# halajun/diasss

Measured on AMD Instinct MI355X. Metric: sonar frames/sec end-to-end (extract+match+LM solve), higher is better.
Workload: dtype u8/int32 (extract, match) + f64 (geo gate, LM); 1 GPU; 200 synthetic 2000x1024 frames, dense all-pairs; frames=200, pings=2000, bins=1024, pairs=19900

## Files before the change

### diasss_amd/csrc/dsss_pg.hip

```cpp
#include "dsss_internal.h"
#include "dsss_lm.h"
#include <utility>
#include "dsss_pg_kernels.h"
#include <algorithm>
#include <numeric>
#include <random>
#include <cstdlib>
#include <chrono>
#include <thread>
#include <mutex>
#include <future>

namespace {

struct pg_dev {
    dsss_ctx* ctx = nullptr;
    int rc = DSSS_OK;
    static constexpr size_t CHUNK = (size_t)256 << 20;
    template <typename T> int alloc(dsss_ctx* c, T** p, size_t n) { void* q = nullptr; if (!rc) rc = grab(c, &q, std::max<size_t>(n, 1) * sizeof(T)); *p = (T*)q; return rc; }
    int grab(dsss_ctx* c, void** p, size_t n) {
        if (!ctx) { ctx = c; c->pg_chunk_cur = 0; c->pg_chunk_off = 0; }
        const size_t bytes = (n + 255) & ~(size_t)255;
        for (;;) {
            if (c->pg_chunk_cur < c->pg_chunks.size()) {
// ... 454 lines not shown
        dv.alloc(c, &d_L, nnzL * 36); dv.alloc(c, &d_ubin, (size_t)S.ubin_doubles);
        if (dv.alloc(c, &d_aval, (size_t)nval * 36 + comm_total)) return dv.rc;
        d_comm = d_aval + (size_t)nval * 36; d_avalif = d_comm; d_xif = d_comm + ncv * 36; d_commU = d_xif + nif * 6;
        if (A.local) ifslot.swap(A.ifslot_g);
        else { ifslot.assign(ns, -1); for (size_t q = 0; q < nif; ++q) ifslot[S.iface_seps[q]] = (int)q; }
        dv.later(&d_ifslot, ifslot); dv.later(&d_ifsep, A.local ? A.ifsep_g : S.iface_seps);
        dv.later(&d_binptr, S.binptr); dv.later(&d_bincols, S.bincols); dv.later(&d_binperm, S.bin_perm);
        dv.later(&d_dest, A.local ? A.dest_g : S.dest_bin);
        dv.later(&d_binroot_ptr, S.binroot_ptr); dv.later(&d_binroot_idx, S.binroot_idx); dv.later(&d_broot_b, S.broot_b); dv.later(&d_broot_uoff, S.broot_uoff);
        dv.later(&d_broot_of_col, S.broot_of_col);
        if (dv.flush(c, st)) return dv.rc;
        { const int nb_all = (int)S.binptr.size() - 1, sel_lo = A.local ? 0 : part_lo, sel_hi = A.local ? 1 : part_hi;
          bin_lo = 0; while (bin_lo < nb_all && S.bin_part[bin_lo] < sel_lo) ++bin_lo; bin_hi = bin_lo; while (bin_hi < nb_all && S.bin_part[bin_hi] < sel_hi) ++bin_hi; }
        nbins = bin_hi - bin_lo;
        return DSSS_OK;
    }
    void bottom_trial(double bins_flops) {
        hipMemsetAsync(d_L, 0, nnzL * 36 * sizeof(double), st);
        if (nparts > 1) hipMemsetAsync(d_comm, 0, comm_total * sizeof(double), st);
        hipLaunchKernelGGL(pg_scatter_base_kernel, dim3((unsigned)(((long long)ns * 78 + 255) / 256)), dim3(256), 0, st, ns, d_t2, d_perm, d_D1, d_g1, d_s2DL, d_s2DR, d_s2GL, d_s2GR, d_s2S, d_dest, d_L, d_aval, d_x,
                           d_ifslot, d_avalif, d_xif, kp0, kp1);
        if (ne > 0) hipLaunchKernelGGL(pg_scatter_lc_kernel, dim3((unsigned)(((long long)ne * 36 + 255) / 256)), dim3(256), 0, st, n, ne, ns, d_Ji, d_ew, d_dest, d_L, d_aval, d_avalif, d_eo, mp0, mp1, d_lc_link);
        if (nbins > 0) { dsss_scope s1(c, DSSS_K_PG_SUBTREE, bins_flops);
                         hipLaunchKernelGGL(pg_factor_subtree_kernel, dim3(nbins), dim3(256), 0, st, d_binperm + bin_lo, d_binptr, d_bincols, d_colptr, d_rlptr, d_rlcol, d_rlpos, d_mapptr, d_map, d_L, d_x, d_fail,
                                            d_binroot_ptr, d_binroot_idx, d_broot_b, d_broot_uoff, d_broot_of_col, d_anc_first, d_anc_rel, d_ubin, d_rdiag); }
    }
    int join_analysis() {
        sym_thread.join();
        if (S.ownership_violations) DSSS_FAIL(c, DSSS_E_STATE, "pose-graph analysis: %d separators with a higher-rank neighbour are not interface", S.ownership_violations);
        return DSSS_OK;
    }

    int upload_fronts() {
        if (!pre_bins) {
            if (const int rc = upload_lists()) return rc;
            if (const int rc = upload_bottom()) return rc;
        } else if (c->prof.on) c->prof.work[DSSS_K_PG_SUBTREE] += std::max(0.0, S.flops_factor - S.flops_fronts);
        if (sw.opt.verbose)
            fprintf(stderr, "[dsss pg] rank %d/%d parts %d (own %d..%d, poses %d..%d)  %s analysis of %d separators  poses %d  LC edges %d  separators %d "
                    "(interface %zu)  nnz(L) blocks %zu  bins %d (%d cols)  fronts %d (largest %d block rows, arena %.0f MB)  panels %d in %d levels  "
                    "all-reduce %.1f MB\n", rank, world, nparts, part_lo, part_hi, mp0, mp1, A.local ? "rank-local" : "replicated", S.ns, n, ne, ns,
                    S.iface_seps.size(), nnzL, (int)S.binptr.size() - 1, (int)S.bincols.size(), (int)S.f_c0.size(), S.max_front_n, S.front_doubles * 8e-6,
                    S.npanels, S.nlev, (S.comm_doubles + 36.0 * S.comm_vals.size() + 6.0 * S.iface_seps.size()) * 8e-6);
        const int nfr = (int)S.f_c0.size();
        f_if = A.local && !S.iface_seps.empty() ? nfr - 1 : -1;
        if_ld = f_if >= 0 ? (size_t)S.f_ld[f_if] : 0; if_count = if_ld * if_ld + if_ld;
        if (f_if >= 0 && (S.f_part[f_if] != -1 || S.f_off[f_if] + (long long)(if_ld * if_ld) != S.front_doubles))
// ... 478 lines not shown
```

### diasss_amd/csrc/dsss_pg_bins.hip

```cpp
#include "dsss_pg_kernels.h"
#include "dsss_pg_dev.h"
#pragma clang fp contract(fast)
__global__ __launch_bounds__(256) void pg_build_map_kernel(int nupd, const int* __restrict__ rlrow, const int* __restrict__ rlptr,
                                                           const int* __restrict__ rlcol, const int* __restrict__ rlpos,
                                                           const int* __restrict__ colptr, const int* __restrict__ rowidx,
                                                           const long long* __restrict__ mapptr, int* __restrict__ upd_map, const int* __restrict__ nupd_dev)
{
    const int e = blockIdx.x * 256 + threadIdx.x;
    if (e >= (nupd_dev ? *nupd_dev : nupd)) return;
    const int j = rlrow[e], k = rlcol[e];
    const int c0 = colptr[j], m = colptr[j + 1] - c0;
    int* mp = upd_map + mapptr[j] + (long long)(e - rlptr[j]) * m;
    int q = 0;
    for (int p = rlpos[e]; p < colptr[k + 1]; ++p) {
        const int i = rowidx[p];
        while (q < m && rowidx[c0 + q] < i) ++q;
        if (q < m && rowidx[c0 + q] == i) mp[q] = p;
    }
}

__global__ __launch_bounds__(256) void pg_rl_count_kernel(int ns, const int* __restrict__ colptr, const int* __restrict__ rowidx, const char* __restrict__ binned,
                                                          int* __restrict__ cnt)
{
    const int k = blockIdx.x * 256 + threadIdx.x;
// ... 99 lines not shown
#pragma unroll
            for (int c = 0; c < 6; ++c) a[u][c] = Lik[c];
        }
#pragma unroll
        for (int u = 0; u < 4; ++u) {
            if (pos[u] < 0) continue;
            const double* B = s_Ljk + (t + u) * 36;
#pragma unroll
            for (int s = 0; s < 6; ++s)
                acc[s] += a[u][0] * B[s * 6] + a[u][1] * B[s * 6 + 1] + a[u][2] * B[s * 6 + 2] + a[u][3] * B[s * 6 + 3] + a[u][4] * B[s * 6 + 4] + a[u][5] * B[s * 6 + 5];
        }
    }
    for (; t < tn; ++t) {
        const int pos = mp[(size_t)t * m];
        if (pos < 0) continue;
        const double* Lik = Lvals + (size_t)pos * 36 + r * 6;
        const double* B = s_Ljk + t * 36;
        const double a0 = Lik[0], a1 = Lik[1], a2 = Lik[2], a3 = Lik[3], a4 = Lik[4], a5 = Lik[5];
#pragma unroll
        for (int s = 0; s < 6; ++s)
            acc[s] += a0 * B[s * 6] + a1 * B[s * 6 + 1] + a2 * B[s * 6 + 2] + a3 * B[s * 6 + 3] + a4 * B[s * 6 + 4] + a5 * B[s * 6 + 5];
    }
}
__global__ __launch_bounds__(256) void pg_factor_subtree_kernel(const int* __restrict__ bin_perm, const int* __restrict__ binptr, const int* __restrict__ bincols,
                                                                const int* __restrict__ colptr, const int* __restrict__ rlptr,
                                                                const int* __restrict__ rlcol, const int* __restrict__ rlpos,
                                                                const long long* __restrict__ mapptr, const int* __restrict__ upd_map,
                                                                double* __restrict__ Lvals, double* __restrict__ x, int* __restrict__ fail,
                                                                const int* __restrict__ binroot_ptr, const int* __restrict__ binroot_idx,
                                                                const int* __restrict__ broot_b, const long long* __restrict__ broot_uoff,
                                                                const int* __restrict__ broot_of_col, const int* __restrict__ anc_first,
                                                                const int* __restrict__ anc_rel, double* __restrict__ ubin, double* __restrict__ rdiag)
{
    __shared__ double s_Ljk[PG_TCH * 36];
    __shared__ double s_yk[PG_TCH * 6];
    __shared__ double s_diag[36];
    __shared__ int s_arel[48];
    __shared__ double s_ri[6];
    __shared__ double s_y[6];
    __shared__ double s_xj[6];
    __shared__ int s_ok;
    const int bin = bin_perm[blockIdx.x];
    for (int q = binroot_ptr[bin]; q < binroot_ptr[bin + 1]; ++q) {
        const int ri = binroot_idx[q]; const long long b6 = 6LL * broot_b[ri]; double* U = ubin + broot_uoff[ri];
        for (long long e = threadIdx.x; e < b6 * b6 + b6; e += 256) U[e] = 0.0;
    }
    struct colinfo { int j, c0, m, t0, T, af, ri, b6; long long mapoff, uoff; };
// ... 105 lines not shown
            double* __restrict__ g = U + (size_t)b6 * b6;
            if ((int)threadIdx.x < ta) s_arel[threadIdx.x] = anc_rel[c0 + af + threadIdx.x];
            __syncthreads();
            if ((int)threadIdx.x < 6 * ta) {
                const int pa = threadIdx.x / 6, a = threadIdx.x - pa * 6;
                const double* La = s_Ljk + pa * 36 + a * 6;
                g[s_arel[pa] * 6 + a] -= La[0] * s_y[0] + La[1] * s_y[1] + La[2] * s_y[2] + La[3] * s_y[3] + La[4] * s_y[4] + La[5] * s_y[5];
            }
            const int npair = ta * (ta + 1) / 2;
            for (int e = threadIdx.x; e < 36 * npair; e += 256) {
                const int pr = e / 36, ab = e - 36 * pr;
                int pa = (int)((sqrtf(8.0f * (float)pr + 1.0f) - 1.0f) * 0.5f);
                while (pa * (pa + 1) / 2 > pr) --pa;
                while ((pa + 1) * (pa + 2) / 2 <= pr) ++pa;
                const int pb = pr - pa * (pa + 1) / 2, a = ab / 6, b = ab - 6 * a;
                const double* La = s_Ljk + pa * 36 + a * 6; const double* Lb = s_Ljk + pb * 36 + b * 6;
                U[(size_t)(s_arel[pa] * 6 + a) * b6 + s_arel[pb] * 6 + b] -= La[0] * Lb[0] + La[1] * Lb[1] + La[2] * Lb[2] + La[3] * Lb[3] + La[4] * Lb[4] + La[5] * Lb[5];
            }
        }
        __syncthreads();
        __threadfence_block();
    }
}
__global__ __launch_bounds__(64) void pg_bwd_subtree_kernel(const int* __restrict__ bin_perm, const int* __restrict__ binptr, const int* __restrict__ bincols,
                                                            const int* __restrict__ colptr, const int* __restrict__ rowidx,
                                                            const double* __restrict__ Lvals, double* __restrict__ x, const double* __restrict__ rdiag)
{
    const int lane = threadIdx.x;
    const int bin = bin_perm[blockIdx.x];
    const int ci_lo = binptr[bin];
    int jn = 0, cn0 = 0, cn1 = 0;
    double ldn[36], rin[6];
    auto ahead = [&](int ci2) {
        jn = bincols[ci2]; cn0 = colptr[jn]; cn1 = colptr[jn + 1];
        if (lane == 0) {
            const double* Ld = Lvals + (size_t)cn0 * 36;
#pragma unroll
            for (int a = 0; a < 36; ++a) ldn[a] = Ld[a];
#pragma unroll
            for (int a = 0; a < 6; ++a) rin[a] = rdiag[(size_t)jn * 6 + a];
        }
    };
    if (binptr[bin + 1] - 1 >= ci_lo) ahead(binptr[bin + 1] - 1);
    for (int ci = binptr[bin + 1] - 1; ci >= ci_lo; --ci) {
        const int j = jn, c0 = cn0, c1 = cn1;
        double ld[36], ri[6];
// ... 36 lines not shown
```

### diasss_amd/csrc/dsss_pg_kernels.h

```cpp
#pragma once
#include "dsss_internal.h"
#include "dsss_pose.h"
#include "dsss_pg_sym.h"

struct pg_weights { double prior[6], odo[6]; };

struct pg_pack { const double* U; const double* g; double* dst; int cld, cb; };
struct pg_front {
    long long off, roff;
    int ld, n6, s6, c0;
    int rowptr, pan0;
    int ch0, ch1, fa0, fa1;
};
struct pg_child { const double* U; const double* g; long long relptr; int cld, cb; };

#define PG_ASM_POSES 32
#define PG_NB4 24
#define PG_RSU_MAX_TILES 320
#define PG_RSU32_MAX_TILES 80
#define PG_BWD2_LD 97
#define PG_BWD2_SX 8192
#define PG_BWD_SPLIT 2048
#define PG_BWD_RC 512
#define RNG_PER_THREAD 16
// ... 16 lines not shown
__global__ void pg_flag_blocksum_kernel(const int* __restrict__ flags, long long n, int* __restrict__ bsum);
__global__ void pg_flag_scan_kernel(int* __restrict__ bsum, int nb, int* __restrict__ total);
__global__ void pg_flag_compact_kernel(const int* __restrict__ flags, const double* __restrict__ pairs, long long n, const int* __restrict__ bsum, long long need_pairs, double* __restrict__ normals);
__global__ void lc_edge_compact_kernel(const int* __restrict__ flags, const int* __restrict__ bsum, const unsigned long long* __restrict__ slot, int total, const int* __restrict__ kp7_off, const double* __restrict__ kp7,
                                       const dsss_lc* __restrict__ lcs, const int* __restrict__ act_s, const int* __restrict__ frame_off, int cap, dsss_lc_edge* __restrict__ edges, int2* __restrict__ ab);
__global__ void pg_gather_dr_kernel(const unsigned long long* __restrict__ fptr, const int* __restrict__ foff, double* __restrict__ out);
__global__ void pg_gather_pose_kernel(int n, const int* __restrict__ idx, const pose_t* __restrict__ X, pose_t* __restrict__ out);
__global__ void pg_sep_xy_kernel(int ns, const int* __restrict__ sep_pose, const double* __restrict__ dr6, double* __restrict__ xy);
__global__ void pg_init_kernel(int n, const double* __restrict__ dr6, const double* __restrict__ normals, int add_noise, pose_t* __restrict__ X, pose_t* __restrict__ meas);
__global__ void pg_rpy_kernel(int n, const pose_t* __restrict__ X, double* __restrict__ rpy6);
__global__ void pg_build_map_kernel(int nupd, const int* __restrict__ rlrow, const int* __restrict__ rlptr, const int* __restrict__ rlcol, const int* __restrict__ rlpos, const int* __restrict__ colptr, const int* __restrict__ rowidx, const long long* __restrict__ mapptr, int* __restrict__ upd_map, const int* __restrict__ nupd_dev);
__global__ void pg_rl_count_kernel(int ns, const int* __restrict__ colptr, const int* __restrict__ rowidx, const char* __restrict__ binned, int* __restrict__ cnt);
template <typename T, int VAL>
__global__ void pg_scan_block_kernel(int n, const int* __restrict__ cnt, const int* __restrict__ colptr, T* __restrict__ out, T* __restrict__ block_sum);
template <typename T>
__global__ void pg_scan_tops_kernel(int nblocks, T* __restrict__ block_sum, T* __restrict__ total);
template <typename T>
__global__ void pg_scan_add_kernel(int n, T* __restrict__ out, const T* __restrict__ block_sum, const T* __restrict__ total);
__global__ void pg_rl_fill_kernel(int ns, const int* __restrict__ colptr, const int* __restrict__ rowidx, const char* __restrict__ binned, const int* __restrict__ rlptr, int* __restrict__ cur, int* __restrict__ rlcol, int* __restrict__ rlpos);
__global__ void pg_rl_sort_kernel(int ns, const int* __restrict__ rlptr, int* __restrict__ rlcol, int* __restrict__ rlpos, int* __restrict__ rlrow, int* __restrict__ fail);
__global__ void pg_fill_map_kernel(int* __restrict__ upd_map, const long long* __restrict__ total);
__global__ void pg_anc_rel_kernel(int ns, const int* __restrict__ colptr, const int* __restrict__ rowidx, const char* __restrict__ binned, const int* __restrict__ root_of, int* __restrict__ anc_first, int* __restrict__ anc_rel);
__global__ void pg_factor_subtree_kernel(const int* __restrict__ bin_perm, const int* __restrict__ binptr, const int* __restrict__ bincols, const int* __restrict__ colptr, const int* __restrict__ rlptr, const int* __restrict__ rlcol, const int* __restrict__ rlpos, const long long* __restrict__ mapptr, const int* __restrict__ upd_map, double* __restrict__ Lvals, double* __restrict__ x, int* __restrict__ fail, const int* __restrict__ binroot_ptr, const int* __restrict__ binroot_idx, const int* __restrict__ broot_b, const long long* __restrict__ broot_uoff, const int* __restrict__ broot_of_col, const int* __restrict__ anc_first, const int* __restrict__ anc_rel, double* __restrict__ ubin, double* __restrict__ rdiag);
__global__ void pg_bwd_subtree_kernel(const int* __restrict__ bin_perm, const int* __restrict__ binptr, const int* __restrict__ bincols, const int* __restrict__ colptr, const int* __restrict__ rowidx, const double* __restrict__ Lvals, double* __restrict__ x, const double* __restrict__ rdiag);
__global__ void pg_front_asm_kernel(const int* __restrict__ it_front, const int* __restrict__ it_row, const pg_front* __restrict__ FD, const pg_child* __restrict__ CH, const int* __restrict__ rel, const int* __restrict__ xr_ptr, const int* __restrict__ xr_child, const int* __restrict__ xr_row, const int* __restrict__ fa_rowptr, const int* __restrict__ fa_src, const int* __restrict__ fa_col, const int* __restrict__ fa_tr, const double* __restrict__ aval, const double* __restrict__ x, double* __restrict__ F, double* __restrict__ R);
__global__ void pg_front_syrk_kernel(const int* __restrict__ it_front, const int* __restrict__ it_step, const pg_front* __restrict__ FD, const int* __restrict__ tile_item, const int* __restrict__ tile_ij, double* __restrict__ F);
__global__ void pg_front_diag4_kernel(const int* __restrict__ it_front, const int* __restrict__ it_step, const pg_front* __restrict__ FD, double* __restrict__ F, double* __restrict__ R, int* __restrict__ fail, double* __restrict__ Tinv);
__global__ void pg_front_trsm2_kernel(const int* __restrict__ it_front, const int* __restrict__ it_step, const pg_front* __restrict__ FD, double* __restrict__ F, double* __restrict__ R, const double* __restrict__ Tinv);
template <int TS>
__global__ void pg_front_rsu_kernel(const int* __restrict__ it_front, const int* __restrict__ it_step, const pg_front* __restrict__ FD, const int* __restrict__ tile_item, const int* __restrict__ tile_ij, double* __restrict__ F, double* __restrict__ FL, double* __restrict__ R, const double* __restrict__ Tinv);
__global__ void pg_front_bwd_part_kernel(const int* __restrict__ it_front, const int* __restrict__ it_step, const pg_front* __restrict__ FD, const int* __restrict__ f_rows, const double* __restrict__ FL, const double* __restrict__ x, double* __restrict__ part, int maxchunks);
__global__ void pg_front_bwd2_kernel(const int* __restrict__ it_front, const int* __restrict__ it_step, const pg_front* __restrict__ FD, const int* __restrict__ f_rows, const double* __restrict__ F, const double* __restrict__ FL, const double* __restrict__ R, double* __restrict__ x, const double* __restrict__ Tinv, const double* __restrict__ part, int maxchunks);
```

### diasss_amd/csrc/dsss_pg_sym.cpp

```cpp
#include "dsss_pg_sym.h"
#include <algorithm>
#include <atomic>
#include <chrono>
#include <condition_variable>
#include <deque>
#include <functional>
#include <cmath>
#include <cstdio>
#include <cstdlib>
#include <cstring>
#include <mutex>
#include <numeric>
#include <thread>

namespace {

class pg_pool {
public:
    struct task { std::function<void()> fn; std::atomic<int> st{ 0 }; };
    static pg_pool& get() { static pg_pool P; return P; }
    void fork(task* t)
    {
        if (workers.empty()) { t->st.store(1); t->fn(); t->st.store(2, std::memory_order_release); return; }
        { std::lock_guard<std::mutex> lk(mu); q.push_back(t); npending.fetch_add(1, std::memory_order_release); }
// ... 1196 lines not shown
    if (opt.on_bottom_ready) opt.on_bottom_ready();
    sym_levels(G);
    sym_row_views(G, std::max(1, opt.threads));
    if (tv) { fprintf(stderr, "[dsss pg symbolic] separators per part:"); for (auto& q : P) fprintf(stderr, " %d", q.nint); fprintf(stderr, "\n"); }
    if (tv) fprintf(stderr, "[dsss pg symbolic] %d parts + an interface of %d: interface %.2f ms, the parts (their graphs, the wait for the coordinates, the analyses; largest %d separators) %.2f ms, joined %.2f ms, levels and row views %.2f ms | ns %d nnzL %lld bins %d fronts %d (max %d rows) panels %d levels %d front arena %.1f MB\n",
                    K, nif, t_pre, [&] { int m = 0; for (auto& q : P) m = std::max(m, q.g.size()); return m; }(), t_parts - t_pre, t_join - t_parts, ms_since(q0) - t_join, ns, G.nnzL,
                    nbG, nfG, G.max_front_n, G.npanels, G.nlev, G.front_doubles * 8e-6);
    return true;
}

}

pg_switches pg_switches_read()
{
    pg_switches sw;
    if (const char* v = getenv("DSSS_PG_BIN_COST")) sw.bin_cost = sw.opt.bin_cost = atof(v);
    if (const char* v = getenv("DSSS_PG_LEAF")) sw.opt.leaf = atoi(v);
    if (const char* v = getenv("DSSS_PG_ND_BOTH")) sw.opt.nd_both_axes = atoi(v);
    if (const char* v = getenv("DSSS_PG_ND_INDEX")) sw.opt.nd_index_cuts = atoi(v);
    if (const char* v = getenv("DSSS_PG_PARTS_ANALYSIS")) sw.parts = atoi(v);
    if (const char* v = getenv("DSSS_SYM_THREADS")) sw.threads = atoi(v);
    if (const char* v = getenv("DSSS_PG_LOCAL")) sw.local = atoi(v) != 0;
    if (const char* v = getenv("DSSS_PG_VERBOSE")) sw.opt.verbose = std::max(1, atoi(v));
    return sw;
}
int pg_cheapest_gap(const int* pos, const std::vector<int>& cross, int target, int width, int after, int* cost)
{
    const int m = (int)cross.size() - 1, lo = std::max(target - width, after + 1);
    auto start = [&](int i) { return pos ? pos[i - 1] + 1 : i; };
    int best = -1; long long bdist = 0;
    for (int i = std::max(1, pos ? (int)(std::lower_bound(pos, pos + m, lo - 1) - pos) + 1 : lo); i < m && start(i) <= target + width; ++i) {
        const long long d = std::llabs((long long)start(i) - target);
        if (best < 0 || cross[i] < *cost || (cross[i] == *cost && d < bdist)) { *cost = cross[i]; bdist = d; best = start(i); }
    }
    return best;
}

void pg_analyse(int ns, const std::vector<std::pair<int, int>>& edges, const double* cx, const double* cy, const int* part, int nparts,
                int part_lo, int part_hi, int world, int rank, const pg_switches& sw, pg_sym_opts opt, pg_analysis& A)
{
    auto sym_threads = [&](int m) { return sw.threads && *sw.threads > 0 ? *sw.threads : (int)std::min(m >= 131072 ? 24u : 8u, std::max(1u, std::thread::hardware_concurrency())); };
    opt.bin_cost = sw.bin_cost.value_or(PG_BIN_COST_DEVICE);
    opt.threads = sym_threads(ns);
    pg_sym& S = A.S;
    if (world > 1 && sw.local) {
        std::vector<int> rank_of_part(nparts, 0), rank_of(ns);
// ... 67 lines not shown
                                  const int32_t* part, int nparts, const double* aval, const double* rhs, double* x, int64_t* stats8)
{
    if (ns < 1 || nedges < ns - 1 || !edge_a || !edge_b || !cx || !cy || (x && (!aval || !rhs))) return DSSS_E_ARG;
    std::vector<std::pair<int, int>> edges;
    if (!twin_edges(ns, edge_a, edge_b, nedges, true, true, edges)) return DSSS_E_ARG;
    pg_sym S;
    const pg_switches sw = pg_switches_read();
    pg_sym_opts opt = sw.opt;
    if (sw.threads) opt.threads = std::max(1, *sw.threads);
    opt.lists_on_device = x == nullptr;
    pg_symbolic(ns, edges, cx, cy, part, nparts, opt, S);
    if (S.ownership_violations) return DSSS_E_STATE;
    if (!x) {
        const auto t0 = std::chrono::steady_clock::now();
        pg_sched so, si; pg_build_schedule(S, 0, std::max(1, nparts), so); if (nparts > 1) pg_build_schedule(S, -1, 0, si);
        if (opt.verbose)
            fprintf(stderr, "[dsss pg symbolic] launch lists %.2f ms (%zu assembly rows, %zu panel steps, %zu tiles)\n",
                    std::chrono::duration<double, std::milli>(std::chrono::steady_clock::now() - t0).count(),
                    so.asmrow_front.size() + si.asmrow_front.size(), so.lv_front.size() + si.lv_front.size(), so.tile_item.size() + si.tile_item.size());
    }
    const int rc = x ? pg_host_solve(S, aval, rhs, x) : 0;
    return twin_result(S, rc, S.comm_doubles, stats8);
}
extern "C" int dsss_host_pg_solve_local(int ns, const int32_t* edge_a, const int32_t* edge_b, int nedges, const double* cx, const double* cy,
                                        const int32_t* iface_last, int nlast, const double* aval, const double* rhs, double* x, int64_t* stats8)
{
    if (ns < 1 || nedges < 0 || (nedges > 0 && (!edge_a || !edge_b)) || !cx || !cy || nlast < 0 || nlast > ns || (nlast > 0 && !iface_last) || !x || !aval || !rhs) return DSSS_E_ARG;
    std::vector<std::pair<int, int>> edges;
    if (!twin_edges(ns, edge_a, edge_b, nedges, false, false, edges)) return DSSS_E_ARG;
    pg_sym S; pg_sym_opts opt = pg_switches_read().opt;
    for (int q = 0; q < nlast; ++q) {
        if (iface_last[q] < 0 || iface_last[q] >= ns || (q > 0 && iface_last[q] <= iface_last[q - 1])) return DSSS_E_ARG;
        opt.iface_last.push_back(iface_last[q]);
    }
    pg_symbolic(ns, edges, cx, cy, nullptr, 1, opt, S);
    if (nlast > 0) {
        const int nf = (int)S.f_c0.size();
        if (!iface_front_last(S, nlast)) return DSSS_E_STATE;
        for (int f = 0; f + 1 < nf; ++f) if (S.f_part[f] < 0) return DSSS_E_STATE;
        for (int q = 0; q < nlast; ++q) if (S.order[ns - nlast + q] != iface_last[q] || (int)S.iface_seps.size() != nlast || S.iface_seps[q] != iface_last[q]) return DSSS_E_STATE;
        if (!S.comm_kind.empty()) return DSSS_E_STATE;
    }
    const int rc = pg_host_solve(S, aval, rhs, x);
    return twin_result(S, rc, (int64_t)S.comm_vals.size(), stats8);
}
extern "C" int dsss_host_pg_solve_parts(int ns, const int32_t* edge_a, const int32_t* edge_b, int nedges, const double* cx, const double* cy,
// ... 13 lines not shown
```

### diasss_amd/csrc/dsss_pg_sym.h

```cpp
#pragma once
#include <functional>
#include <optional>
#include <vector>

void dsss_pool_run(int T, const std::function<void(int)>& fn);

#define PG_PW 16
#define PG_PARTS_CUT_MAX 12
#define PG_PARTS_IFACE_MAX 256
#define PG_LOCAL_IFACE_MAX 160

constexpr double PG_BIN_COST_HOST = 1000, PG_BIN_COST_DEVICE = 600, PG_BIN_COST_RANK = 120;

struct pg_sym {
    int ns = 0, nparts = 1;
    std::vector<int> perm;
    std::vector<int> order;
    std::vector<int> colptr, rowidx;
    std::vector<int> parent;
    std::vector<int> col_part;
    std::vector<char> binned;
    std::vector<int> binptr, bincols;
    std::vector<int> bin_part;
    std::vector<double> bin_work;
// ... 51 lines not shown
    int leaf = 24;
    int nd_both_axes = 64;
    int nd_index_cuts = 1;
    bool nd_geo_first = true;
    double bin_cost = PG_BIN_COST_HOST;
    double pack_cost = 0;
    int threads = 4;
    double relax_zero_blocks = 8, relax_flops = 1.05, relax_flops_small = 1.6;
    double relax_abs_flops = 0;
    std::function<void()> on_bottom_ready;
    std::function<void()> on_lists_ready;
    bool lists_on_device = false;
    std::function<void()> before_order;
    std::vector<int> iface_last;
    bool to_be_joined = false;
    int verbose = 0;
};

struct pg_switches {
    pg_sym_opts opt;
    std::optional<double> bin_cost;
    std::optional<int> parts, threads;
    bool local = true;
};
pg_switches pg_switches_read();

int pg_cheapest_gap(const int* pos, const std::vector<int>& cross, int target, int width, int after, int* cost);

struct pg_analysis {
    pg_sym S;
    pg_sched SO, SI;
    bool local = false;
    std::vector<int> perm_g, dest_g, ifslot_g, ifsep_g;
};
void pg_analyse(int ns, const std::vector<std::pair<int, int>>& edges, const double* cx, const double* cy, const int* part, int nparts,
                int part_lo, int part_hi, int world, int rank, const pg_switches& sw, pg_sym_opts opt, pg_analysis& A);
```

### include/dsss.h

```cpp
#ifndef DSSS_H
#define DSSS_H

#include <stdint.h>
#include <stddef.h>

#ifdef __cplusplus
extern "C" {
#endif

#define DSSS_OK            0
#define DSSS_E_NODEVICE   -1
#define DSSS_E_ARG        -2
#define DSSS_E_HIP        -3
#define DSSS_E_STATE      -4
#define DSSS_E_CAPACITY   -5
#define DSSS_E_NUMERIC    -6
#define DSSS_E_COMM       -7

typedef struct dsss_ctx dsss_ctx;

typedef struct { float x, y, size, angle, response; int32_t octave; } dsss_kp;

typedef struct {
    double factor;  int32_t width, r, side;
// ... 94 lines not shown
int dsss_posegraph_update(dsss_ctx*, int nframes, double* poses12_host, double* rpy6_host, double* stats4_host);
int dsss_posegraph_update_window(dsss_ctx*, int nframes, int window_frames, double* poses12_host, double* rpy6_host, double* stats4_host);
int dsss_posegraph_reset(dsss_ctx*);
int dsss_posegraph_online_edges(dsss_ctx*);
int dsss_posegraph_schedule_get(dsss_ctx*, int* levels4_host, int cap_levels, int* n_levels, int* n_trials);
int dsss_posegraph_solve_edges(dsss_ctx*, const double* dr6, int total, const dsss_lc_edge* edges, int ne,
                               double* poses12_host, double* stats4_host);

int dsss_posegraph_edge_report(dsss_ctx*, const double* dr6, int total, const dsss_lc_edge* edges, int ne,
                               const double* poses12, double* chi2_host, double* r6_host, double* sums3_host);

typedef struct { double gate, decade; int32_t max_solves, pad_; } dsss_pg_gate_params;
void dsss_pg_gate_params_default(dsss_pg_gate_params*);
int dsss_posegraph_solve_gated(dsss_ctx*, const double* dr6, int total, const dsss_lc_edge* edges, int ne,
                               const dsss_pg_gate_params*, double* poses12_host, double* stats4_host,
                               uint8_t* keep_host , double* chi2_host , int* n_solves_host);

int dsss_host_pg_solve(int ns, const int32_t* edge_a, const int32_t* edge_b, int nedges, const double* cx, const double* cy,
                       const int32_t* part, int nparts, const double* aval36, const double* rhs6, double* x6_host, int64_t* stats8);
int dsss_host_pg_solve_local(int ns, const int32_t* edge_a, const int32_t* edge_b, int nedges, const double* cx, const double* cy,
                             const int32_t* iface_last, int nlast, const double* aval36, const double* rhs6, double* x6_host, int64_t* stats8);
int dsss_host_pg_solve_parts(int ns, const int32_t* edge_a, const int32_t* edge_b, int nedges, const double* cx, const double* cy,
                             int K, const double* aval36, const double* rhs6, double* x6_host, int64_t* stats8);

typedef struct { double x0, y0, cell; int32_t W, H; int32_t use_mask; int32_t pad_; } dsss_mosaic_params;
int dsss_mosaic_grid(const double* bbox4, double cell, dsss_mosaic_params* out);
int dsss_mosaic_bounds(dsss_ctx*, const int* ids, int n, const double* rpy6, const int* ping_off, double* bbox4_host);
int dsss_mosaic_render(dsss_ctx*, const int* ids, int n, const double* rpy6, const int* ping_off,
                       const dsss_mosaic_params*, uint32_t* sum_host, uint32_t* cnt_host, uint8_t* img_host);
int dsss_mosaic_consistency(dsss_ctx*, const int* ids, int n, const double* rpy6, const int* ping_off,
                            const dsss_mosaic_params*, uint32_t* nfr_host, uint32_t* s1_host, uint32_t* s2_host,
                            double* score_host);

typedef struct { int32_t radius, min_cells; } dsss_reg_params;
typedef struct { int32_t dx, dy; double off_x, off_y;
                 double zncc, zncc0; int64_t n, n0;
                 int32_t on_border, pad_; } dsss_reg_result;
void dsss_reg_params_default(dsss_reg_params*);
int  dsss_mosaic_register(dsss_ctx*, const int* ids, int n, const double* rpy6, const int* ping_off, const dsss_mosaic_params*,
                          const int* pair_a, const int* pair_b, int npairs, const dsss_reg_params*,
                          dsss_reg_result* out_host , uint64_t* sums_host );
int  dsss_mosaic_register_peak(const uint64_t* sums, int radius, int min_cells, double cell, dsss_reg_result* out);

typedef struct { int32_t pair, seg, p0, p1;
                 dsss_reg_result r;
                 int64_t sx, sy; } dsss_reg_seg;
// ... 46 lines not shown
```

Measured before the change: 9570 frames/s.

## Software-pipeline the subtree factor kernel across consecutive columns in a bin

Rewrites the per-bin subtree Cholesky kernel so it prefetches the next column's update rows and map indices and starts accumulating them while the current column's diagonal is factored, using double-buffered shared staging. It also caches column descriptors in shared memory with wave-uniform reads and keeps the previous column's block in shared memory to skip a global reload. The old kernel stays reachable as a serial variant through an environment switch, and a host profiling entry point for bin statistics is added. The kernel becomes more complex, uses more shared memory and registers (launch bounds of 256 threads with 3 blocks), and only benefits the pose-graph part of the end-to-end pipeline.

```diff
diff --git a/diasss_amd/csrc/dsss_pg.hip b/diasss_amd/csrc/dsss_pg.hip
--- a/diasss_amd/csrc/dsss_pg.hip
+++ b/diasss_amd/csrc/dsss_pg.hip
@@ -500,7 +500,7 @@
                            d_ifslot, d_avalif, d_xif, kp0, kp1);
         if (ne > 0) hipLaunchKernelGGL(pg_scatter_lc_kernel, dim3((unsigned)(((long long)ne * 36 + 255) / 256)), dim3(256), 0, st, n, ne, ns, d_Ji, d_ew, d_dest, d_L, d_aval, d_avalif, d_eo, mp0, mp1, d_lc_link);
         if (nbins > 0) { dsss_scope s1(c, DSSS_K_PG_SUBTREE, bins_flops);
-                         hipLaunchKernelGGL(pg_factor_subtree_kernel, dim3(nbins), dim3(256), 0, st, d_binperm + bin_lo, d_binptr, d_bincols, d_colptr, d_rlptr, d_rlcol, d_rlpos, d_mapptr, d_map, d_L, d_x, d_fail,
+                         hipLaunchKernelGGL(sw.bins_serial ? pg_factor_subtree_serial_kernel : pg_factor_subtree_kernel, dim3(nbins), dim3(256), 0, st, d_binperm + bin_lo, d_binptr, d_bincols, d_colptr, d_rlptr, d_rlcol, d_rlpos, d_mapptr, d_map, d_L, d_x, d_fail,
                                             d_binroot_ptr, d_binroot_idx, d_broot_b, d_broot_uoff, d_broot_of_col, d_anc_first, d_anc_rel, d_ubin, d_rdiag); }
     }
     int join_analysis() {
diff --git a/diasss_amd/csrc/dsss_pg_bins.hip b/diasss_amd/csrc/dsss_pg_bins.hip
--- a/diasss_amd/csrc/dsss_pg_bins.hip
+++ b/diasss_amd/csrc/dsss_pg_bins.hip
@@ -145,7 +145,7 @@
             acc[s] += a0 * B[s * 6] + a1 * B[s * 6 + 1] + a2 * B[s * 6 + 2] + a3 * B[s * 6 + 3] + a4 * B[s * 6 + 4] + a5 * B[s * 6 + 5];
     }
 }
-__global__ __launch_bounds__(256) void pg_factor_subtree_kernel(const int* __restrict__ bin_perm, const int* __restrict__ binptr, const int* __restrict__ bincols,
+__global__ __launch_bounds__(256) void pg_factor_subtree_serial_kernel(const int* __restrict__ bin_perm, const int* __restrict__ binptr, const int* __restrict__ bincols,
                                                                 const int* __restrict__ colptr, const int* __restrict__ rlptr,
                                                                 const int* __restrict__ rlcol, const int* __restrict__ rlpos,
                                                                 const long long* __restrict__ mapptr, const int* __restrict__ upd_map,
@@ -297,6 +297,291 @@
         __threadfence_block();
     }
 }
+#define PG_PCH 42
+#define PG_NIDX 4
+#define PG_DW 64
+struct pg_coldesc { int j, c0, m, t0, T, af, ri, b6, fpos, c0p; long long mapoff, uoff; };
+__device__ inline void pg_upd_term(double (&acc)[6], const double (&a)[6], const double* __restrict__ B)
+{
+#pragma unroll
+    for (int s = 0; s < 6; ++s)
+        acc[s] += a[0] * B[s * 6] + a[1] * B[s * 6 + 1] + a[2] * B[s * 6 + 2] + a[3] * B[s * 6 + 3] + a[4] * B[s * 6 + 4] + a[5] * B[s * 6 + 5];
+}
+__device__ inline void pg_upd_group(const int (&pos)[4], int t, const double* __restrict__ Lvals, int r, const double* __restrict__ s_B, double (&acc)[6])
+{
+    double a[4][6];
+#pragma unroll
+    for (int u = 0; u < 4; ++u) {
+        const double* Lik = Lvals + (size_t)(pos[u] < 0 ? 0 : pos[u]) * 36 + r * 6;
+#pragma unroll
+        for (int c = 0; c < 6; ++c) a[u][c] = Lik[c];
+    }
+#pragma unroll
+    for (int u = 0; u < 4; ++u) {
+        if (pos[u] < 0) continue;
+        pg_upd_term(acc, a[u], s_B + (t + u) * 36);
+    }
+}
+__device__ inline void pg_acc_rows_ahead(const int (&mpi)[PG_NIDX], const int* __restrict__ mp, int m, int tn, const double* __restrict__ Lvals, int r,
+                                         const double* __restrict__ s_B, double (&acc)[6])
+{
+    const int ng = (tn + 3) >> 2;
+#pragma unroll
+    for (int g = 0; g < PG_NIDX / 4; ++g)
+        if (g < ng) {
+            int pos[4];
+#pragma unroll
+            for (int u = 0; u < 4; ++u) pos[u] = 4 * g + u < tn ? mpi[4 * g + u] : -1;
+            pg_upd_group(pos, 4 * g, Lvals, r, s_B, acc);
+        }
+    for (int g = PG_NIDX / 4; g < ng; ++g) {
+        int pos[4];
+#pragma unroll
+        for (int u = 0; u < 4; ++u) pos[u] = mp[(size_t)min(4 * g + u, tn - 1) * m];
+#pragma unroll
+        for (int u = 0; u < 4; ++u) if (4 * g + u >= tn) pos[u] = -1;
+        pg_upd_group(pos, 4 * g, Lvals, r, s_B, acc);
+    }
+}
+__global__ __launch_bounds__(256, 3) void pg_factor_subtree_kernel(const int* __restrict__ bin_perm, const int* __restrict__ binptr, const int* __restrict__ bincols,
+                                                                const int* __restrict__ colptr, const int* __restrict__ rlptr,
+                                                                const int* __restrict__ rlcol, const int* __restrict__ rlpos,
+                                                                const long long* __restrict__ mapptr, const int* __restrict__ upd_map,
+                                                                double* __restrict__ Lvals, double* __restrict__ x, int* __restrict__ fail,
+                                                                const int* __restrict__ binroot_ptr, const int* __restrict__ binroot_idx,
+                                                                const int* __restrict__ broot_b, const long long* __restrict__ broot_uoff,
+                                                                const int* __restrict__ broot_of_col, const int* __restrict__ anc_first,
+                                                                const int* __restrict__ anc_rel, double* __restrict__ ubin, double* __restrict__ rdiag)
+{
+    __shared__ double s_st[2][PG_PCH * 36];
+    __shared__ double s_sy[2][PG_PCH * 6];
+    __shared__ double s_col[42 * 36];
+    __shared__ double s_diag[36];
+    __shared__ double s_ri[6];
+    __shared__ double s_y[2][6];
+    __shared__ int s_arel[2][48];
+    __shared__ int s_di[PG_DW][10];
+    __shared__ long long s_dl[PG_DW][2];
+    __shared__ double s_xj[6];
+    __shared__ int s_ok;
+    const int tid = threadIdx.x;
+    const int bin = bin_perm[blockIdx.x];
+    for (int q = binroot_ptr[bin]; q < binroot_ptr[bin + 1]; ++q) {
+        const int ri = binroot_idx[q]; const long long b6 = 6LL * broot_b[ri]; double* U = ubin + broot_uoff[ri];
+        for (long long e = threadIdx.x; e < b6 * b6 + b6; e += 256) U[e] = 0.0;
+    }
+    const int ci0 = binptr[bin], ci_end = binptr[bin + 1];
+    if (ci0 >= ci_end) return;
+    auto fill = [&](int base, int cnt) {
+        if (tid < cnt) {
+            const int ci = base + tid, j = bincols[ci];
+            const int c0 = colptr[j], m = colptr[j + 1] - c0, t0 = rlptr[j], T = rlptr[j + 1] - t0, ri = broot_of_col[j];
+            int fpos = -1, c0p = 0;
+            if (ci > ci0 && T > 0) {
+                const int jp = bincols[ci - 1];
+                if (rlcol[t0 + T - 1] == jp) { c0p = colptr[jp]; fpos = rlpos[t0 + T - 1] - c0p; }
+            }
+            int* d = s_di[(ci - ci0) & (PG_DW - 1)];
+            d[0] = j; d[1] = c0; d[2] = m; d[3] = t0; d[4] = T; d[5] = anc_first[j]; d[6] = ri; d[7] = ri >= 0 ? 6 * broot_b[ri] : 0; d[8] = fpos; d[9] = c0p;
+            long long* dl = s_dl[(ci - ci0) & (PG_DW - 1)];
+            dl[0] = mapptr[j]; dl[1] = ri >= 0 ? broot_uoff[ri] : 0;
+        }
+    };
+    auto desc = [&](int ci) {
+        const int* d = s_di[(ci - ci0) & (PG_DW - 1)]; const long long* dl = s_dl[(ci - ci0) & (PG_DW - 1)];
+        pg_coldesc k;
+        k.j = __builtin_amdgcn_readfirstlane(d[0]); k.c0 = __builtin_amdgcn_readfirstlane(d[1]); k.m = __builtin_amdgcn_readfirstlane(d[2]);
+        k.t0 = __builtin_amdgcn_readfirstlane(d[3]); k.T = __builtin_amdgcn_readfirstlane(d[4]); k.af = __builtin_amdgcn_readfirstlane(d[5]);
+        k.ri = __builtin_amdgcn_readfirstlane(d[6]); k.b6 = __builtin_amdgcn_readfirstlane(d[7]); k.fpos = __builtin_amdgcn_readfirstlane(d[8]);
+        k.c0p = __builtin_amdgcn_readfirstlane(d[9]);
+        const long long mo = dl[0], uo = dl[1];
+        k.mapoff = ((long long)__builtin_amdgcn_readfirstlane((int)(mo >> 32)) << 32) | (unsigned)__builtin_amdgcn_readfirstlane((int)mo);
+        k.uoff = ((long long)__builtin_amdgcn_readfirstlane((int)(uo >> 32)) << 32) | (unsigned)__builtin_amdgcn_readfirstlane((int)uo);
+        return k;
+    };
+    auto u_update = [&](const pg_coldesc& k, const double* sy, const int* sa) {
+        const int ta = k.m - k.af;
+        if (k.ri < 0 || ta <= 0) return;
+        const int b6 = k.b6;
+        double* __restrict__ U = ubin + k.uoff;
+        double* __restrict__ g = U + (size_t)b6 * b6;
+        const double* sL = s_col + k.af * 36;
+        if (tid < 6 * ta) {
+            const int pa = tid / 6, a = tid - pa * 6;
+            const double* La = sL + pa * 36 + a * 6;
+            g[sa[pa] * 6 + a] -= La[0] * sy[0] + La[1] * sy[1] + La[2] * sy[2] + La[3] * sy[3] + La[4] * sy[4] + La[5] * sy[5];
+        }
+        const int npair = ta * (ta + 1) / 2;
+        for (int it = tid; it < 6 * npair; it += 256) {
+            const int pr = it / 6, a = it - 6 * pr;
+            int pa = (int)((sqrtf(8.0f * (float)pr + 1.0f) - 1.0f) * 0.5f);
+            while (pa * (pa + 1) / 2 > pr) --pa;
+            while ((pa + 1) * (pa + 2) / 2 <= pr) ++pa;
+            const int pb = pr - pa * (pa + 1) / 2;
+            const double* La = sL + pa * 36 + a * 6;
+            double* Ur = U + (size_t)(sa[pa] * 6 + a) * b6 + sa[pb] * 6;
+            double old[6];
+#pragma unroll
+            for (int b = 0; b < 6; ++b) old[b] = Ur[b];
+            const double la[6] = { La[0], La[1], La[2], La[3], La[4], La[5] };
+#pragma unroll
+            for (int b = 0; b < 6; ++b) {
+                const double* Lb = sL + pb * 36 + b * 6;
+                Ur[b] = old[b] - (la[0] * Lb[0] + la[1] * Lb[1] + la[2] * Lb[2] + la[3] * Lb[3] + la[4] * Lb[4] + la[5] * Lb[5]);
+            }
+        }
+    };
+    fill(ci0, min(PG_DW, ci_end - ci0));
+    __syncthreads();
+    const int q = tid / 6, r = tid - q * 6;
+    const bool rhs = tid >= 250;
+    const int rs_ = rhs ? tid - 250 : 0;
+    pg_coldesc cur = desc(ci0), prv = cur;
+    double acc[6] = { 0, 0, 0, 0, 0, 0 }, accy = 0, rowv[6] = { 0, 0, 0, 0, 0, 0 }, xa = 0;
+    const int* idle = bin_perm + blockIdx.x;
+    int mpf = -1, arel, ip, ic;
+#pragma unroll
+    for (int s = 0; s < 6; ++s) rowv[s] = Lvals[(size_t)(cur.c0 + (tid < 6 * cur.m ? q : 0)) * 36 + r * 6 + s];
+    xa = x[(size_t)cur.j * 6 + rs_];
+    arel = *(tid < cur.m - cur.af ? anc_rel + cur.c0 + cur.af + tid : idle);
+    {
+        const pg_coldesc d1 = ci0 + 1 < ci_end ? desc(ci0 + 1) : cur;
+        const bool st1 = ci0 + 1 < ci_end && tid < 6 * min(PG_PCH, d1.T - (d1.fpos >= 0));
+        ip = *(st1 ? rlpos + d1.t0 + q : idle); ic = *(st1 ? rlcol + d1.t0 + q : idle);
+    }
+    for (int ci = ci0; ci < ci_end; ++ci) {
+        const int par = ci & 1, rel = ci - ci0;
+        const bool have1 = ci + 1 < ci_end, have2 = ci + 2 < ci_end;
+        if (rel >= 32 && (rel & 31) == 0 && ci + 32 < ci_end) fill(ci + 32, min(32, ci_end - (ci + 32)));
+        const pg_coldesc d1 = have1 ? desc(ci + 1) : cur;
+        const int m = cur.m, c0 = cur.c0, j = cur.j;
+        const bool act = tid < 6 * m;
+        const int Tnf = cur.T - (cur.fpos >= 0);
+        const int* mp = upd_map + cur.mapoff;
+        const int Tnf1 = have1 ? d1.T - (d1.fpos >= 0) : 0, tn1 = min(PG_PCH, Tnf1);
+        const bool act1 = have1 && tid < 6 * d1.m;
+        const int* mp1 = upd_map + d1.mapoff;
+        int mpi[PG_NIDX], mpf1, arel1, ip2, ic2;
+#pragma unroll
+        for (int u = 0; u < PG_NIDX; ++u) mpi[u] = *(act1 && u < tn1 ? mp1 + (size_t)u * d1.m + q : idle);
+        mpf1 = *(act1 && d1.fpos >= 0 ? mp1 + (size_t)(d1.T - 1) * d1.m + q : idle);
+        arel1 = *(have1 && tid < d1.m - d1.af ? anc_rel + d1.c0 + d1.af + tid : idle);
+        double sv[6], syv;
+        {
+            const bool st1 = tid < 6 * tn1;
+            const size_t ipc = st1 ? ip : 0, icc = st1 ? ic : 0;
+#pragma unroll
+            for (int s = 0; s < 6; ++s) sv[s] = Lvals[ipc * 36 + r * 6 + s];
+            syv = x[icc * 6 + r];
+        }
+        {
+            const pg_coldesc d2 = have2 ? desc(ci + 2) : cur;
+            const bool st2 = have2 && tid < 6 * min(PG_PCH, d2.T - (d2.fpos >= 0));
+            ip2 = *(st2 ? rlpos + d2.t0 + q : idle); ic2 = *(st2 ? rlcol + d2.t0 + q : idle);
+        }
+        for (int tc = ci == ci0 ? 0 : min(PG_PCH, Tnf); tc < Tnf; tc += PG_PCH) {
+            const int tn = min(PG_PCH, Tnf - tc);
+            __syncthreads();
+            if (tid < 6 * tn) {
+                const int pos = rlpos[cur.t0 + tc + q], col = rlcol[cur.t0 + tc + q];
+#pragma unroll
+                for (int s = 0; s < 6; ++s) s_st[par][tid * 6 + s] = Lvals[(size_t)pos * 36 + r * 6 + s];
+                s_sy[par][tid] = x[(size_t)col * 6 + r];
+            }
+            __syncthreads();
+            if (rhs)
+                for (int t = 0; t < tn; ++t) {
+                    const double* yk = s_sy[par] + t * 6; const double* B = s_st[par] + t * 36 + rs_ * 6;
+                    accy += B[0] * yk[0] + B[1] * yk[1] + B[2] * yk[2] + B[3] * yk[3] + B[4] * yk[4] + B[5] * yk[5];
+                }
+            if (act) pg_acc_rows(mp + (size_t)tc * m + q, m, tn, Lvals, r, s_st[par], acc);
+        }
+        if (cur.fpos >= 0) {
+            const double* Bf = s_col + cur.fpos * 36;
+            if (rhs) {
+                const double* yk = s_y[par ^ 1]; const double* B = Bf + rs_ * 6;
+                accy += B[0] * yk[0] + B[1] * yk[1] + B[2] * yk[2] + B[3] * yk[3] + B[4] * yk[4] + B[5] * yk[5];
+            }
+            if (act && mpf >= 0) {
+                const double* Lik = s_col + (mpf - cur.c0p) * 36 + r * 6;
+                const double a[6] = { Lik[0], Lik[1], Lik[2], Lik[3], Lik[4], Lik[5] };
+                pg_upd_term(acc, a, Bf);
+            }
+        }
+        if (rhs) s_xj[rs_] = xa - accy;
+        if (act) {
+#pragma unroll
+            for (int s = 0; s < 6; ++s) rowv[s] -= acc[s];
+            if (tid < 6) { for (int s = 0; s < 6; ++s) s_diag[r * 6 + s] = rowv[s]; }
+        }
+        if (tid < m - cur.af) s_arel[par][tid] = arel;
+        if (tid < 6 * tn1) {
+#pragma unroll
+            for (int s = 0; s < 6; ++s) s_st[par ^ 1][tid * 6 + s] = sv[s];
+            s_sy[par ^ 1][tid] = syv;
+        }
+        __syncthreads();
+        double acc1[6] = { 0, 0, 0, 0, 0, 0 }, accy1 = 0, rowv1[6] = { 0, 0, 0, 0, 0, 0 }, xa1 = 0;
+        if (tid == 250) {
+            double A[36], xj[6], ri[6];
+#pragma unroll
+            for (int a = 0; a < 36; ++a) A[a] = s_diag[a];
+#pragma unroll
+            for (int a = 0; a < 6; ++a) xj[a] = s_xj[a];
+            const int bad = chol6_recip(A, ri);
+            if (bad) *fail = 1;
+            s_ok = !bad;
+#pragma unroll
+            for (int a = 0; a < 6; ++a)
+#pragma unroll
+                for (int b = 0; b < 6; ++b) { const double v = b <= a ? A[a * 6 + b] : 0.0; s_diag[a * 6 + b] = v; Lvals[(size_t)c0 * 36 + a * 6 + b] = v; }
+#pragma unroll
+            for (int a = 0; a < 6; ++a) { s_ri[a] = ri[a]; rdiag[(size_t)j * 6 + a] = ri[a]; }
+            if (!bad) {
+                double v[6];
+#pragma unroll
+                for (int a = 0; a < 6; ++a) {
+                    double t = xj[a];
+#pragma unroll
+                    for (int b = 0; b < 6; ++b) if (b < a) t -= A[a * 6 + b] * v[b];
+                    v[a] = t * ri[a];
+                }
+#pragma unroll
+                for (int a = 0; a < 6; ++a) { x[(size_t)j * 6 + a] = v[a]; s_y[par][a] = v[a]; }
+            }
+        }
+        if (ci > ci0) u_update(prv, s_y[par ^ 1], s_arel[par ^ 1]);
+        if (tn1 > 0) {
+            if (rhs)
+                for (int t = 0; t < tn1; ++t) {
+                    const double* yk = s_sy[par ^ 1] + t * 6; const double* B = s_st[par ^ 1] + t * 36 + rs_ * 6;
+                    accy1 += B[0] * yk[0] + B[1] * yk[1] + B[2] * yk[2] + B[3] * yk[3] + B[4] * yk[4] + B[5] * yk[5];
+                }
+            if (act1) pg_acc_rows_ahead(mpi, mp1 + q, d1.m, tn1, Lvals, r, s_st[par ^ 1], acc1);
+        }
+#pragma unroll
+        for (int s = 0; s < 6; ++s) rowv1[s] = Lvals[(size_t)(d1.c0 + (act1 ? q : 0)) * 36 + r * 6 + s];
+        xa1 = x[(size_t)d1.j * 6 + rs_];
+        __syncthreads();
+        if (!s_ok) return;
+        if (act && tid >= 6) {
+            double* row = Lvals + (size_t)(c0 + q) * 36 + r * 6;
+            double xr[6];
+#pragma unroll
+            for (int s = 0; s < 6; ++s) { double v = rowv[s];
+#pragma unroll
+                                          for (int c = 0; c < 6; ++c) if (c < s) v -= xr[c] * s_diag[s * 6 + c];
+                                          xr[s] = v * s_ri[s]; }
+            for (int s = 0; s < 6; ++s) { row[s] = xr[s]; s_col[tid * 6 + s] = xr[s]; }
+        }
+        __syncthreads();
+        prv = cur; cur = d1;
+#pragma unroll
+        for (int s = 0; s < 6; ++s) { acc[s] = acc1[s]; rowv[s] = rowv1[s]; }
+        accy = accy1; xa = xa1; mpf = mpf1; arel = arel1; ip = ip2; ic = ic2;
+    }
+    u_update(prv, s_y[(ci_end - 1) & 1], s_arel[(ci_end - 1) & 1]);
+}
 __global__ __launch_bounds__(64) void pg_bwd_subtree_kernel(const int* __restrict__ bin_perm, const int* __restrict__ binptr, const int* __restrict__ bincols,
                                                             const int* __restrict__ colptr, const int* __restrict__ rowidx,
                                                             const double* __restrict__ Lvals, double* __restrict__ x, const double* __restrict__ rdiag)
diff --git a/diasss_amd/csrc/dsss_pg_kernels.h b/diasss_amd/csrc/dsss_pg_kernels.h
--- a/diasss_amd/csrc/dsss_pg_kernels.h
+++ b/diasss_amd/csrc/dsss_pg_kernels.h
@@ -62,6 +62,7 @@
 __global__ void pg_fill_map_kernel(int* __restrict__ upd_map, const long long* __restrict__ total);
 __global__ void pg_anc_rel_kernel(int ns, const int* __restrict__ colptr, const int* __restrict__ rowidx, const char* __restrict__ binned, const int* __restrict__ root_of, int* __restrict__ anc_first, int* __restrict__ anc_rel);
 __global__ void pg_factor_subtree_kernel(const int* __restrict__ bin_perm, const int* __restrict__ binptr, const int* __restrict__ bincols, const int* __restrict__ colptr, const int* __restrict__ rlptr, const int* __restrict__ rlcol, const int* __restrict__ rlpos, const long long* __restrict__ mapptr, const int* __restrict__ upd_map, double* __restrict__ Lvals, double* __restrict__ x, int* __restrict__ fail, const int* __restrict__ binroot_ptr, const int* __restrict__ binroot_idx, const int* __restrict__ broot_b, const long long* __restrict__ broot_uoff, const int* __restrict__ broot_of_col, const int* __restrict__ anc_first, const int* __restrict__ anc_rel, double* __restrict__ ubin, double* __restrict__ rdiag);
+__global__ void pg_factor_subtree_serial_kernel(const int* __restrict__ bin_perm, const int* __restrict__ binptr, const int* __restrict__ bincols, const int* __restrict__ colptr, const int* __restrict__ rlptr, const int* __restrict__ rlcol, const int* __restrict__ rlpos, const long long* __restrict__ mapptr, const int* __restrict__ upd_map, double* __restrict__ Lvals, double* __restrict__ x, int* __restrict__ fail, const int* __restrict__ binroot_ptr, const int* __restrict__ binroot_idx, const int* __restrict__ broot_b, const long long* __restrict__ broot_uoff, const int* __restrict__ broot_of_col, const int* __restrict__ anc_first, const int* __restrict__ anc_rel, double* __restrict__ ubin, double* __restrict__ rdiag);
 __global__ void pg_bwd_subtree_kernel(const int* __restrict__ bin_perm, const int* __restrict__ binptr, const int* __restrict__ bincols, const int* __restrict__ colptr, const int* __restrict__ rowidx, const double* __restrict__ Lvals, double* __restrict__ x, const double* __restrict__ rdiag);
 __global__ void pg_front_asm_kernel(const int* __restrict__ it_front, const int* __restrict__ it_row, const pg_front* __restrict__ FD, const pg_child* __restrict__ CH, const int* __restrict__ rel, const int* __restrict__ xr_ptr, const int* __restrict__ xr_child, const int* __restrict__ xr_row, const int* __restrict__ fa_rowptr, const int* __restrict__ fa_src, const int* __restrict__ fa_col, const int* __restrict__ fa_tr, const double* __restrict__ aval, const double* __restrict__ x, double* __restrict__ F, double* __restrict__ R);
 __global__ void pg_front_syrk_kernel(const int* __restrict__ it_front, const int* __restrict__ it_step, const pg_front* __restrict__ FD, const int* __restrict__ tile_item, const int* __restrict__ tile_ij, double* __restrict__ F);
diff --git a/diasss_amd/csrc/dsss_pg_sym.cpp b/diasss_amd/csrc/dsss_pg_sym.cpp
--- a/diasss_amd/csrc/dsss_pg_sym.cpp
+++ b/diasss_amd/csrc/dsss_pg_sym.cpp
@@ -1242,6 +1242,7 @@
     if (const char* v = getenv("DSSS_SYM_THREADS")) sw.threads = atoi(v);
     if (const char* v = getenv("DSSS_PG_LOCAL")) sw.local = atoi(v) != 0;
     if (const char* v = getenv("DSSS_PG_VERBOSE")) sw.opt.verbose = std::max(1, atoi(v));
+    if (const char* v = getenv("DSSS_PG_BINS")) sw.bins_serial = strcmp(v, "serial") == 0;
     return sw;
 }
 int pg_cheapest_gap(const int* pos, const std::vector<int>& cross, int target, int width, int after, int* cost)
@@ -1355,6 +1356,43 @@
     const int rc = x ? pg_host_solve(S, aval, rhs, x) : 0;
     return twin_result(S, rc, S.comm_doubles, stats8);
 }
+extern "C" int dsss_host_pg_bins_profile(int ns, const int32_t* edge_a, const int32_t* edge_b, int nedges, const double* cx, const double* cy, int64_t* prof12)
+{
+    if (ns < 1 || nedges < ns - 1 || !edge_a || !edge_b || !cx || !cy || !prof12) return DSSS_E_ARG;
+    std::vector<std::pair<int, int>> edges;
+    if (!twin_edges(ns, edge_a, edge_b, nedges, true, true, edges)) return DSSS_E_ARG;
+    pg_sym S;
+    const pg_switches sw = pg_switches_read();
+    pg_sym_opts opt = sw.opt;
+    if (sw.threads) opt.threads = std::max(1, *sw.threads);
+    opt.bin_cost = sw.bin_cost.value_or(PG_BIN_COST_DEVICE);
+    pg_symbolic(ns, edges, cx, cy, nullptr, 1, opt, S);
+    int64_t* p = prof12;
+    for (int k = 0; k < 12; ++k) p[k] = 0;
+    const int nb = (int)S.binptr.size() - 1;
+    p[0] = nb; p[1] = (int64_t)S.bincols.size();
+    for (int b = 0; b < nb; ++b) {
+        const int lo = S.binptr[b], hi = S.binptr[b + 1];
+        if (hi - lo == 1) ++p[2];
+        p[8] = std::max<int64_t>(p[8], S.binroot_ptr[b + 1] - S.binroot_ptr[b]);
+        p[10] = std::max<int64_t>(p[10], hi - lo);
+        for (int ci = lo; ci < hi; ++ci) {
+            const int j = S.bincols[ci], T = S.rlptr[j + 1] - S.rlptr[j], m = S.colptr[j + 1] - S.colptr[j];
+            bool fresh = false;
+            if (ci > lo) {
+                const int jp = S.bincols[ci - 1], Tp = S.rlptr[jp + 1] - S.rlptr[jp];
+                fresh = T > 0 && S.rlcol[S.rlptr[j + 1] - 1] == jp;
+                if (T == 0 && Tp > 0) ++p[3];
+                if (fresh) ++p[4]; else if (T > 0) ++p[5];
+                if (S.broot_of_col[j] >= 0 && S.broot_of_col[j] == S.broot_of_col[jp] && m - S.anc_first[j] > 0 && S.colptr[jp + 1] - S.colptr[jp] - S.anc_first[jp] > 0) ++p[9];
+            }
+            p[6] = std::max<int64_t>(p[6], T - (fresh ? 1 : 0));
+            p[7] = std::max<int64_t>(p[7], m);
+            p[11] = std::max<int64_t>(p[11], T);
+        }
+    }
+    return DSSS_OK;
+}
 extern "C" int dsss_host_pg_solve_local(int ns, const int32_t* edge_a, const int32_t* edge_b, int nedges, const double* cx, const double* cy,
                                         const int32_t* iface_last, int nlast, const double* aval, const double* rhs, double* x, int64_t* stats8)
 {
diff --git a/diasss_amd/csrc/dsss_pg_sym.h b/diasss_amd/csrc/dsss_pg_sym.h
--- a/diasss_amd/csrc/dsss_pg_sym.h
+++ b/diasss_amd/csrc/dsss_pg_sym.h
@@ -97,6 +97,7 @@
     std::optional<double> bin_cost;
     std::optional<int> parts, threads;
     bool local = true;
+    bool bins_serial = false;
 };
 pg_switches pg_switches_read();
 
diff --git a/include/dsss.h b/include/dsss.h
--- a/include/dsss.h
+++ b/include/dsss.h
@@ -140,6 +140,7 @@
                              const int32_t* iface_last, int nlast, const double* aval36, const double* rhs6, double* x6_host, int64_t* stats8);
 int dsss_host_pg_solve_parts(int ns, const int32_t* edge_a, const int32_t* edge_b, int nedges, const double* cx, const double* cy,
                              int K, const double* aval36, const double* rhs6, double* x6_host, int64_t* stats8);
+int dsss_host_pg_bins_profile(int ns, const int32_t* edge_a, const int32_t* edge_b, int nedges, const double* cx, const double* cy, int64_t* prof12);
 
 typedef struct { double x0, y0, cell; int32_t W, H; int32_t use_mask; int32_t pad_; } dsss_mosaic_params;
 int dsss_mosaic_grid(const double* bbox4, double cell, dsss_mosaic_params* out);
```

Measured after the change: 9811 frames/s (median of 6 runs). 2.5% higher.
